# zhm1205/Multimodal_TTA

Measured on AMD Instinct MI355X. Metric: adapted volumes/sec, higher is better.
Workload: dtype bf16

## Files before the change

include/mmtta.h:

```cpp
#ifndef MMTTA_H
#define MMTTA_H

#include <stdint.h>

#ifdef __cplusplus
extern "C" {
#endif

#define MMTTA_ABI_VERSION 2

typedef enum {
  MMTTA_OK = 0,
  MMTTA_ERR_INVALID = -1,
  MMTTA_ERR_UNSUPPORTED = -2,
  MMTTA_ERR_LAUNCH = -3,
  MMTTA_ERR_WORKSPACE = -4
} mmtta_status;

typedef enum { MMTTA_F32 = 0, MMTTA_BF16 = 1 } mmtta_dtype;

typedef struct {
  void* ptr;
  int32_t n, c, d, h, w;
  int64_t sn, sc, sd, sh, sw;
// ... 9 lines not shown
typedef struct {
  const float* mean;
  const float* rstd;
  const float* gamma;
  const float* beta;
  int32_t relu;
  int32_t per_item;
  const float* scale;
  const float* shift;
  float negative_slope;
  int32_t _pad2;
} mmtta_norm_on_load;

const char* mmtta_last_error(void);
int mmtta_abi_version(void);

#define MMTTA_OPT_PROFILE_MAIN_KERNEL_ONLY 1
#define MMTTA_OPT_SPLITK_BELOW 2
#define MMTTA_OPT_SPLITK_TARGET 3
#define MMTTA_OPT_WGRAD_WORKGROUPS 4
#define MMTTA_OPT_WGRAD_THIN_SLABS 5
#define MMTTA_OPT_IGEMM_PIPELINE 6
#define MMTTA_OPT_EPILOGUE_VEC16 9
#define MMTTA_OPT_IGEMM_LEAN 10
#define MMTTA_OPT_WGRAD_VECTOR_STAGING 11
#define MMTTA_OPT_CLASS_FUSED_MIN_WORKGROUPS 12
#define MMTTA_OPT_THIN_MFMA 13
#define MMTTA_OPT_IGEMM_FRAGMENT_REUSE 14
#define MMTTA_OPT_LAME_TILED 15
#define MMTTA_OPT_RAW_STAGING 16
#define MMTTA_OPT_HEAD_LOSS_PAIR 17
#define MMTTA_OPT_THIN_LEAN 18
#define MMTTA_OPT_WGRAD_EPILOGUE_UPDATE 19
int mmtta_set_option(int key, int value);

int mmtta_copy_strided(const mmtta_tensor* src, const mmtta_tensor* dst, void* stream);

typedef enum {
  MMTTA_CONV_FWD = 0,
  MMTTA_CONV_DGRAD = 1,
  MMTTA_CONVT_FWD = 2,
  MMTTA_CONVT_DGRAD = 3
} mmtta_conv_op;

typedef struct {
  int32_t op;
  int32_t ksize;
  int32_t stride;
  int32_t cin;
  int32_t cout;
  int32_t dtype;
} mmtta_conv_desc;

int64_t mmtta_conv_packed_bytes(const mmtta_conv_desc* desc);

int mmtta_conv_pack_weights(const mmtta_conv_desc* desc, const float* w_master, void* packed, void* stream);

typedef struct {
  mmtta_conv_desc desc;
  const float* w_master;
  void* packed;
} mmtta_pack_item;
int64_t mmtta_conv_pack_table_bytes(int count);
int mmtta_conv_pack_table_build(const mmtta_pack_item* items, int count, void* table_host, int64_t* total);
int mmtta_conv_pack_batched(const void* table_dev, int count, int64_t total, void* stream);

typedef struct {
  int32_t tiles;
  int32_t launches;
  int32_t ksplit;
  int32_t stats_rows;
  int32_t config;
  int32_t _pad;
  int64_t workspace_bytes;
} mmtta_conv_plan_t;

int mmtta_conv_plan(const mmtta_conv_desc* desc, const mmtta_tensor* x, const mmtta_tensor* y,
                    mmtta_conv_plan_t* plan);

typedef struct {
  const mmtta_tensor* add;
  mmtta_norm_on_load add_norm;
} mmtta_conv_epilogue;

int mmtta_conv_run(const mmtta_conv_desc* desc, const mmtta_tensor* x, const mmtta_norm_on_load* x_norm,
                   const void* packed, const float* bias, const mmtta_conv_epilogue* epi,
                   const mmtta_tensor* y, int accumulate, float* stats, void* workspace,
                   int64_t workspace_bytes, void* stream);

int mmtta_conv_route(const mmtta_conv_desc* desc, const mmtta_tensor* x, const mmtta_norm_on_load* x_norm,
                     const mmtta_conv_epilogue* epi, const mmtta_tensor* y, int accumulate, const float* stats);

int mmtta_conv_stages_raw(const mmtta_conv_desc* desc, const mmtta_tensor* x, const mmtta_norm_on_load* x_norm,
                          const mmtta_conv_epilogue* epi, const mmtta_tensor* y, int accumulate, const float* stats);

int mmtta_conv_thin_lean(const mmtta_conv_desc* desc, const mmtta_tensor* x, const mmtta_norm_on_load* x_norm,
                         const mmtta_conv_epilogue* epi, const mmtta_tensor* y, int accumulate, const float* stats);

typedef struct {
  int32_t items_per_set;
  int32_t inner;
  int64_t packed_outer, packed_inner;
  int64_t weight_outer, weight_inner;
  int64_t bias_outer, bias_inner;
} mmtta_param_sets;

int mmtta_conv_run_sets(const mmtta_conv_desc* desc, const mmtta_tensor* x, const mmtta_norm_on_load* x_norm,
                        const void* packed, const float* bias, const mmtta_conv_epilogue* epi,
                        const mmtta_tensor* y, int accumulate, float* stats, void* workspace,
                        int64_t workspace_bytes, const mmtta_param_sets* sets, void* stream);

int mmtta_conv_head_loss_eligible(const mmtta_conv_desc* desc, const mmtta_tensor* x, const mmtta_norm_on_load* x_norm,
                                  const mmtta_conv_epilogue* epi, const mmtta_tensor* y, const mmtta_tensor* dlogits,
                                  int softmax, int per_item);
int64_t mmtta_conv_head_loss_partials(const mmtta_conv_desc* desc, const mmtta_tensor* x, const mmtta_tensor* y);
int mmtta_conv_head_loss_run_sets(const mmtta_conv_desc* desc, const mmtta_tensor* x, const mmtta_norm_on_load* x_norm,
                                  const void* packed, const float* bias, const mmtta_conv_epilogue* epi,
                                  const mmtta_tensor* y, const mmtta_tensor* dlogits, int softmax, int per_item,
                                  double* partial, float* loss, const mmtta_param_sets* sets, void* stream);

int64_t mmtta_conv_wgrad_workspace_bytes(const mmtta_conv_desc* desc, const mmtta_tensor* x,
                                         const mmtta_tensor* dy);
int mmtta_conv_wgrad_kernel(const mmtta_conv_desc* desc, const mmtta_tensor* x, const mmtta_tensor* dy);
int mmtta_conv_wgrad_stages_raw(const mmtta_conv_desc* desc, const mmtta_tensor* x, const mmtta_norm_on_load* x_norm,
                                const mmtta_tensor* dy);
int mmtta_conv_wgrad(const mmtta_conv_desc* desc, const mmtta_tensor* x, const mmtta_norm_on_load* x_norm,
                     const mmtta_tensor* dy, float* dw, float* db, int accumulate, void* workspace,
// ... 319 lines not shown
```

multimodal_tta_amd/_lib.py:

```python
from __future__ import annotations

import ctypes as C
import os
from typing import Optional, Sequence

import torch

_HERE = os.path.dirname(os.path.abspath(__file__))
LIB_PATH = os.path.join(_HERE, "csrc", "libmmtta.so")

F32, BF16 = 0, 1
CONV_FWD, CONV_DGRAD, CONVT_FWD, CONVT_DGRAD = 0, 1, 2, 3
NORM_INSTANCE, NORM_BATCH, NORM_GROUP = 0, 1, 2


class MmttaError(RuntimeError):
    pass


class Tensor(C.Structure):
    _fields_ = [
        ("ptr", C.c_void_p),
        ("n", C.c_int32), ("c", C.c_int32), ("d", C.c_int32), ("h", C.c_int32), ("w", C.c_int32),
        ("sn", C.c_int64), ("sc", C.c_int64), ("sd", C.c_int64), ("sh", C.c_int64), ("sw", C.c_int64),
# ... 73 lines not shown


class IntensityRule(C.Structure):
    _fields_ = [("clip", C.c_int32), ("zscore", C.c_int32), ("masked", C.c_int32), ("min_count", C.c_int32),
                ("lo", C.c_float), ("hi", C.c_float), ("mask_gt", C.c_float), ("eps", C.c_float),
                ("mean", C.c_float), ("std", C.c_float), ("legacy", C.c_int32), ("_pad", C.c_int32)]


class InputNormBranch(C.Structure):
    _fields_ = [("dy", C.POINTER(Tensor)), ("weight", C.c_void_p), ("set_stride", C.c_int64), ("ksize", C.c_int32),
                ("stride", C.c_int32)]


_P = C.POINTER
_SIGNATURES = {
    "mmtta_last_error": (C.c_char_p, []),
    "mmtta_abi_version": (C.c_int, []),
    "mmtta_set_option": (C.c_int, [C.c_int, C.c_int]),
    "mmtta_intensity_scratch_bytes": (C.c_int64, [C.c_int]),
    "mmtta_intensity_normalize": (C.c_int, [_P(Tensor), _P(IntensityRule), _P(Tensor), C.c_void_p, C.c_void_p]),
    "mmtta_copy_strided": (C.c_int, [_P(Tensor), _P(Tensor), C.c_void_p]),
    "mmtta_conv_packed_bytes": (C.c_int64, [_P(ConvDesc)]),
    "mmtta_conv_pack_weights": (C.c_int, [_P(ConvDesc), C.c_void_p, C.c_void_p, C.c_void_p]),
    "mmtta_conv_pack_table_bytes": (C.c_int64, [C.c_int]),
    "mmtta_conv_pack_table_build": (C.c_int, [_P(PackItem), C.c_int, C.c_void_p, _P(C.c_int64)]),
    "mmtta_conv_pack_batched": (C.c_int, [C.c_void_p, C.c_int, C.c_int64, C.c_void_p]),
    "mmtta_conv_plan": (C.c_int, [_P(ConvDesc), _P(Tensor), _P(Tensor), _P(ConvPlan)]),
    "mmtta_conv_run": (C.c_int, [_P(ConvDesc), _P(Tensor), _P(NormOnLoad), C.c_void_p, C.c_void_p, _P(ConvEpilogue),
                                 _P(Tensor), C.c_int, C.c_void_p, C.c_void_p, C.c_int64, C.c_void_p]),
    "mmtta_conv_run_sets": (C.c_int, [_P(ConvDesc), _P(Tensor), _P(NormOnLoad), C.c_void_p, C.c_void_p, _P(ConvEpilogue),
                                      _P(Tensor), C.c_int, C.c_void_p, C.c_void_p, C.c_int64, _P(ParamSets), C.c_void_p]),
    "mmtta_conv_route": (C.c_int, [_P(ConvDesc), _P(Tensor), _P(NormOnLoad), _P(ConvEpilogue), _P(Tensor), C.c_int, C.c_void_p]),
    "mmtta_conv_stages_raw": (C.c_int, [_P(ConvDesc), _P(Tensor), _P(NormOnLoad), _P(ConvEpilogue), _P(Tensor), C.c_int, C.c_void_p]),
    "mmtta_conv_thin_lean": (C.c_int, [_P(ConvDesc), _P(Tensor), _P(NormOnLoad), _P(ConvEpilogue), _P(Tensor), C.c_int, C.c_void_p]),
    "mmtta_conv_head_loss_eligible": (C.c_int, [_P(ConvDesc), _P(Tensor), _P(NormOnLoad), _P(ConvEpilogue), _P(Tensor), _P(Tensor),
                                                C.c_int, C.c_int]),
    "mmtta_conv_head_loss_partials": (C.c_int64, [_P(ConvDesc), _P(Tensor), _P(Tensor)]),
    "mmtta_conv_head_loss_run_sets": (C.c_int, [_P(ConvDesc), _P(Tensor), _P(NormOnLoad), C.c_void_p, C.c_void_p, _P(ConvEpilogue),
                                                _P(Tensor), _P(Tensor), C.c_int, C.c_int, C.c_void_p, C.c_void_p, _P(ParamSets),
                                                C.c_void_p]),
    "mmtta_conv_wgrad_workspace_bytes": (C.c_int64, [_P(ConvDesc), _P(Tensor), _P(Tensor)]),
    "mmtta_conv_wgrad_workspace_bytes_sets": (C.c_int64, [_P(ConvDesc), _P(Tensor), _P(Tensor), _P(ParamSets)]),
    "mmtta_conv_wgrad_plan_sets": (C.c_int, [_P(ConvDesc), _P(Tensor), _P(Tensor), _P(ParamSets), _P(C.c_int32)]),
    "mmtta_conv_wgrad_sets": (C.c_int, [_P(ConvDesc), _P(Tensor), _P(NormOnLoad), _P(Tensor), C.c_void_p, C.c_void_p,
                                        C.c_int, C.c_void_p, C.c_int64, _P(ParamSets), C.c_void_p]),
    "mmtta_conv_wgrad_kernel": (C.c_int, [_P(ConvDesc), _P(Tensor), _P(Tensor)]),
    "mmtta_conv_wgrad_stages_raw": (C.c_int, [_P(ConvDesc), _P(Tensor), _P(NormOnLoad), _P(Tensor)]),
    "mmtta_conv_wgrad": (C.c_int, [_P(ConvDesc), _P(Tensor), _P(NormOnLoad), _P(Tensor), C.c_void_p, C.c_void_p,
                                   C.c_int, C.c_void_p, C.c_int64, C.c_void_p]),
    "mmtta_norm_stats_finalize": (C.c_int, [C.c_int, C.c_int, C.c_void_p, C.c_int, C.c_int, C.c_int, C.c_int64,
                                            C.c_float, C.c_int, C.c_void_p, C.c_void_p, C.c_float, C.c_void_p,
                                            C.c_void_p, C.c_void_p, C.c_void_p, C.c_void_p, C.c_void_p, C.c_void_p,
                                            C.c_void_p]),
    "mmtta_norm_stats_finalize_sets": (C.c_int, [C.c_int, C.c_int, C.c_void_p, C.c_int, C.c_int, C.c_int, C.c_int64,
                                                 C.c_float, C.c_int, C.c_void_p, C.c_void_p, C.c_float, C.c_void_p,
                                                 C.c_void_p, C.c_void_p, C.c_void_p, C.c_void_p, C.c_void_p, C.c_void_p,
                                                 C.c_void_p, C.c_void_p, _P(NormSets), C.c_void_p]),
    "mmtta_reduce_rows_per_n": (C.c_int, [_P(Tensor)]),
    "mmtta_channel_stats": (C.c_int, [_P(Tensor), C.c_void_p, C.c_void_p]),
    "mmtta_combine": (C.c_int, [_P(Tensor), _P(NormOnLoad), _P(Tensor), _P(NormOnLoad), _P(Tensor), C.c_void_p]),
    "mmtta_norm_bwd_reduce": (C.c_int, [_P(Tensor), _P(Tensor), _P(NormOnLoad), C.c_void_p, C.c_void_p]),
    "mmtta_norm_bwd_finalize": (C.c_int, [C.c_int, C.c_int, C.c_void_p, C.c_int, C.c_int, C.c_int, C.c_int64,
                                          C.c_void_p, C.c_int, C.c_void_p, C.c_void_p, C.c_void_p, C.c_void_p,
                                          C.c_int, C.c_void_p, C.c_void_p]),
    "mmtta_norm_bwd_finalize_sets": (C.c_int, [C.c_int, C.c_int, C.c_void_p, C.c_int, C.c_int, C.c_int, C.c_int64,
                                               C.c_void_p, C.c_int, C.c_void_p, C.c_void_p, C.c_void_p, C.c_void_p,
# ... 128 lines not shown
        return _lib
    if not os.path.exists(LIB_PATH):
        raise MmttaError(
            f"{LIB_PATH} is missing: build it with `python -m multimodal_tta_amd.build` (hipcc, gfx950). "
            "There is no CPU or PyTorch fallback for the adaptation path."
        )
    lib = C.CDLL(LIB_PATH)
    for name, (res, args) in _SIGNATURES.items():
        fn = getattr(lib, name)
        fn.restype = res
        fn.argtypes = args
    if lib.mmtta_abi_version() != 2:
        raise MmttaError("libmmtta.so ABI version mismatch")
    if os.environ.get("MMTTA_NO_PIPE", "0") == "1":
        lib.mmtta_set_option(6, 0)
    if os.environ.get("MMTTA_NO_EPIVEC", "0") == "1":
        lib.mmtta_set_option(9, 0)
    if "MMTTA_WGVEC" in os.environ:
        lib.mmtta_set_option(11, int(os.environ["MMTTA_WGVEC"]))
    if "MMTTA_THINMFMA" in os.environ:
        lib.mmtta_set_option(13, int(os.environ["MMTTA_THINMFMA"]))
    if "MMTTA_CLSFUSE" in os.environ:
        lib.mmtta_set_option(12, int(os.environ["MMTTA_CLSFUSE"]))
    if "MMTTA_LEAN" in os.environ:
        lib.mmtta_set_option(10, int(os.environ["MMTTA_LEAN"]))
    if "MMTTA_RAWSTAGE" in os.environ:
        lib.mmtta_set_option(16, int(os.environ["MMTTA_RAWSTAGE"]))
    if "MMTTA_HEADLOSS" in os.environ:
        lib.mmtta_set_option(17, int(os.environ["MMTTA_HEADLOSS"]))
    if "MMTTA_THINLEAN" in os.environ:
        lib.mmtta_set_option(18, int(os.environ["MMTTA_THINLEAN"]))
    if "MMTTA_EPIUPDATE" in os.environ:
        lib.mmtta_set_option(19, int(os.environ["MMTTA_EPIUPDATE"]))
    _lib = lib
    return lib


def exported_names() -> Sequence[str]:
    return list(_SIGNATURES)


def check(status: int, what: str = "") -> None:
    if status != 0:
        msg = load().mmtta_last_error().decode("utf-8", "replace")
        raise MmttaError(f"{what or 'libmmtta'} failed with status {status}: {msg}")


def stream_ptr() -> int:
    return int(torch.cuda.current_stream().cuda_stream)


def ptr(t: Optional[torch.Tensor]) -> Optional[int]:
    return None if t is None else int(t.data_ptr())


TENSOR_OWNS_PAD = 1


def desc_cl(t: torch.Tensor) -> Tensor:
    if t.dim() != 5 or t.dtype not in (torch.float32, torch.bfloat16) or not t.is_cuda:
        raise MmttaError(f"expected a CUDA float32 / bfloat16 [N,D,H,W,C] view, got {tuple(t.shape)} {t.dtype} {t.device}")
    n, d, h, w, c = t.shape
    sn, sd, sh, sw, sc = t.stride()
    if sc != 1 and c != 1:
        raise MmttaError("activation views must have unit stride along C")
    flags = TENSOR_OWNS_PAD if getattr(t, "_mmtta_owns_pad", False) else 0
# ... 20 lines not shown
```

multimodal_tta_amd/csrc/api.hip:

```cpp
#include "common.h"
#include <string.h>

namespace mmtta {
static thread_local char g_err[512] = "";
void set_error(const char* fmt, ...) {
  va_list ap;
  va_start(ap, fmt);
  vsnprintf(g_err, sizeof(g_err), fmt, ap);
  va_end(ap);
}
int g_profile_main_only = 0;
int g_igemm_pipeline = 1;
int g_epilogue_vec = 1;
int g_igemm_lean = 1;
int g_igemm_reuse = 1;
int g_cls_fused_min = 128;
int g_thin_mfma = 2;
int g_wgrad_vec = 1;
int g_lame_tiled = 1;
int g_raw_staging = 3;
int g_head_loss_pair = 3;
int g_thin_lean = 3;
int g_wgrad_epilogue_update = 1;
int g_tune[4] = {96, 128, 128, 256};
}

extern "C" int mmtta_set_option(int key, int value) {
  if (key == MMTTA_OPT_PROFILE_MAIN_KERNEL_ONLY) {
    const int prev = mmtta::g_profile_main_only;
    mmtta::g_profile_main_only = value;
    return prev;
  }
  if (key == MMTTA_OPT_WGRAD_VECTOR_STAGING) {
    const int prev = mmtta::g_wgrad_vec;
    mmtta::g_wgrad_vec = value ? 1 : 0;
    return prev;
  }
  if (key == MMTTA_OPT_THIN_MFMA) {
    const int prev = mmtta::g_thin_mfma;
    mmtta::g_thin_mfma = value < 0 ? 0 : (value > 3 ? 3 : value);
    return prev;
  }
  if (key == MMTTA_OPT_CLASS_FUSED_MIN_WORKGROUPS) {
    const int prev = mmtta::g_cls_fused_min;
    mmtta::g_cls_fused_min = value < 0 ? 0 : value;
    return prev;
  }
  if (key == MMTTA_OPT_IGEMM_LEAN) {
    const int prev = mmtta::g_igemm_lean;
    mmtta::g_igemm_lean = value ? 1 : 0;
    return prev;
  }
  if (key == MMTTA_OPT_IGEMM_FRAGMENT_REUSE) {
    const int prev = mmtta::g_igemm_reuse;
    mmtta::g_igemm_reuse = value ? 1 : 0;
    return prev;
  }
  if (key == MMTTA_OPT_EPILOGUE_VEC16) {
    const int prev = mmtta::g_epilogue_vec;
    mmtta::g_epilogue_vec = value ? 1 : 0;
    return prev;
  }
  if (key == MMTTA_OPT_LAME_TILED) {
    const int prev = mmtta::g_lame_tiled;
    mmtta::g_lame_tiled = value ? 1 : 0;
    return prev;
  }
  if (key == MMTTA_OPT_RAW_STAGING) {
    const int prev = mmtta::g_raw_staging;
    mmtta::g_raw_staging = value & 3;
    return prev;
  }
  if (key == MMTTA_OPT_HEAD_LOSS_PAIR) {
    const int prev = mmtta::g_head_loss_pair;
    mmtta::g_head_loss_pair = value & 3;
    return prev;
  }
  if (key == MMTTA_OPT_THIN_LEAN) {
    const int prev = mmtta::g_thin_lean;
    mmtta::g_thin_lean = value & 3;
    return prev;
  }
  if (key == MMTTA_OPT_WGRAD_EPILOGUE_UPDATE) {
    const int prev = mmtta::g_wgrad_epilogue_update;
    mmtta::g_wgrad_epilogue_update = value ? 1 : 0;
    return prev;
  }
  if (key == MMTTA_OPT_IGEMM_PIPELINE) {
    const int prev = mmtta::g_igemm_pipeline;
    mmtta::g_igemm_pipeline = value ? 1 : 0;
    return prev;
  }
  if (key >= MMTTA_OPT_SPLITK_BELOW && key <= MMTTA_OPT_WGRAD_THIN_SLABS) {
    if (value < 1) return MMTTA_ERR_INVALID;
    const int prev = mmtta::g_tune[key - MMTTA_OPT_SPLITK_BELOW];
    mmtta::g_tune[key - MMTTA_OPT_SPLITK_BELOW] = value;
    return prev;
  }
  return MMTTA_ERR_INVALID;
}

extern "C" const char* mmtta_last_error(void) { return mmtta::g_err; }
extern "C" int mmtta_abi_version(void) { return MMTTA_ABI_VERSION; }
```

multimodal_tta_amd/csrc/common.h:

```cpp
#pragma once
#include <hip/hip_runtime.h>
#include <type_traits>
#include <stdint.h>
#include <stdio.h>
#include <stdarg.h>
#include "../../include/mmtta.h"

namespace mmtta {

constexpr int WAVE = 64;

void set_error(const char* fmt, ...);

#define MMTTA_CHECK(cond, code, ...)      \
  do {                                    \
    if (!(cond)) {                        \
      ::mmtta::set_error(__VA_ARGS__);    \
      return (code);                      \
    }                                     \
  } while (0)

inline int launch_status(const char* what) {
  hipError_t e = hipGetLastError();
  if (e != hipSuccess) {
    set_error("%s: %s", what, hipGetErrorString(e));
    return MMTTA_ERR_LAUNCH;
  }
  return MMTTA_OK;
}

extern int g_profile_main_only;
extern int g_igemm_pipeline;
extern int g_wgrad_vec;
extern int g_igemm_lean;
extern int g_igemm_reuse;
extern int g_cls_fused_min;
extern int g_lame_tiled;
extern int g_thin_mfma;
extern int g_epilogue_vec;
extern int g_raw_staging;
extern int g_head_loss_pair;
extern int g_thin_lean;
extern int g_wgrad_epilogue_update;
extern int g_tune[4];

inline bool nl_leaky(const mmtta_norm_on_load* t) { return t != nullptr && t->relu == MMTTA_ACT_LEAKY_RELU; }
inline int nl_act_check(const mmtta_norm_on_load* t, const char* what) {
  MMTTA_CHECK(t == nullptr || (t->relu >= MMTTA_ACT_NONE && t->relu <= MMTTA_ACT_LEAKY_RELU), MMTTA_ERR_INVALID,
              "%s: activation code %d (MMTTA_ACT_NONE, _RELU or _LEAKY_RELU)", what, t ? t->relu : 0);
  MMTTA_CHECK(t == nullptr || t->relu != MMTTA_ACT_LEAKY_RELU || __builtin_isfinite(t->negative_slope), MMTTA_ERR_INVALID,
              "%s: LeakyReLU negative_slope must be finite", what);
  return MMTTA_OK;
}

struct PackImageGeo {
  int A, B, T, Kp, Np, kn_is_ba, plain_bf16;
};
int pack_image_geometry(const mmtta_conv_desc* d, PackImageGeo& g);

#define MMTTA_ACT_BODIES                                                                                                    \
  int conv_run_body(const mmtta_conv_desc* d, const mmtta_tensor* x, const mmtta_norm_on_load* x_norm, const void* packed,  \
                    const float* bias, const mmtta_conv_epilogue* epi, const mmtta_tensor* y, int accumulate, float* stats, \
                    void* workspace, int64_t workspace_bytes, const mmtta_param_sets* sets, void* stream);                \
  int conv_wgrad_body(const mmtta_conv_desc* d, const mmtta_tensor* x, const mmtta_norm_on_load* x_norm,                    \
                      const mmtta_tensor* dy, float* dw, float* db, int accumulate, void* workspace,                        \
                      int64_t workspace_bytes, const mmtta_param_sets* sets, void* stream,                                  \
                      const mmtta_update_target* upd);                                                                      \
  int combine_body(const mmtta_tensor* a, const mmtta_norm_on_load* ta, const mmtta_tensor* b,                              \
                   const mmtta_norm_on_load* tb, const mmtta_tensor* out, void* stream);                                    \
  int norm_bwd_reduce_body(const mmtta_tensor* dout, const mmtta_tensor* y, const mmtta_norm_on_load* t, float* part,      \
                           void* stream);                                                                                   \
  int norm_bwd_apply_body(const mmtta_tensor* dout, const mmtta_tensor* y, const mmtta_norm_on_load* t, const float* m1,   \
                          const float* m2, const mmtta_tensor* dy, void* stream);                                           \
  int norm_bwd_small_body(const mmtta_tensor* dout, const mmtta_tensor* y, const mmtta_norm_on_load* t, int64_t count,     \
                          const mmtta_tensor* dy, void* stream);
namespace leaky { MMTTA_ACT_BODIES }
// ... 460 lines not shown
```

multimodal_tta_amd/csrc/conv_igemm.hip:

```cpp
#include "common.h"

namespace mmtta {
MMTTA_ACT_NS_OPEN

typedef float f32x16 __attribute__((ext_vector_type(16)));
typedef __bf16 bf16x8 __attribute__((ext_vector_type(8)));
typedef __bf16 bf16x2 __attribute__((ext_vector_type(2)));

__device__ __forceinline__ unsigned int pack_bf16x2(float lo, float hi) {
  bf16x2 v;
  v[0] = (__bf16)lo;
  v[1] = (__bf16)hi;
  return __builtin_bit_cast(unsigned int, v);
}

struct Taps {
  int n;
  int slab[27];
  signed char dz[27], dy[27], dx[27];
  int zmin, ymin, xmin;
  int zext, yext, xext;
};

struct ClassInfo {
// ... 217 lines not shown
}

template <int NB, int MB, int TZ, int TY, int TX, int KCI, int OCC>
__global__ __launch_bounds__(256, OCC) void igemm_raw_kernel(GArgs a) {
  constexpr bool BF = true, ABF = true, REUSE = false, RAW = true;
#include "conv_igemm_body.h"
}

template <bool ABF>
__global__ __launch_bounds__(256, 3) void igemm_reuse_raw_kernel(GArgs a) {
  constexpr int NB = 1, MB = 2, TZ = 4, TY = 8, TX = 8, KCI = 16, OCC = 3;
  constexpr bool BF = true, REUSE = true, RAW = true;
#include "conv_igemm_body.h"
}

struct ClsTap { int cls, d, slab; };
__host__ __device__ constexpr ClsTap cls_tap(int f) {
  int idx = 0;
  for (int cls = 0; cls < 8; ++cls) {
    const int pz = (cls >> 2) & 1, py = (cls >> 1) & 1, px = cls & 1;
    for (int a = 0; a <= pz; ++a)
      for (int b = 0; b <= py; ++b)
        for (int c = 0; c <= px; ++c) {
          const int kz = pz ? (a == 0 ? 0 : 2) : 1, dz = pz ? (a == 0 ? 1 : 0) : 0;
          const int ky = py ? (b == 0 ? 0 : 2) : 1, dy = py ? (b == 0 ? 1 : 0) : 0;
          const int kx = px ? (c == 0 ? 0 : 2) : 1, dx = px ? (c == 0 ? 1 : 0) : 0;
          if (idx == f) return ClsTap{cls, (dz * 2 + dy) * 2 + dx, (kz * 3 + ky) * 3 + kx};
          ++idx;
        }
  }
  return ClsTap{0, 0, 0};
}

template <int KCI, bool ABF>
__global__ __launch_bounds__(256, 2) void igemm_cls8_kernel(GArgs a) {
  constexpr bool RAW = false;
#include "conv_igemm_cls8_body.h"
}

template <int KCI, bool ABF>
__global__ __launch_bounds__(256, 2) void igemm_cls8_raw_kernel(GArgs a) {
  constexpr bool RAW = true;
#include "conv_igemm_cls8_body.h"
}

template <int KCI, bool ABF, bool RAW = false>
static int launch_cls8_t(const GArgs& a, int tiles, hipStream_t s) {
  constexpr int VS = KCI + 8;
  size_t lds = ((size_t)(5 * 5 * LDS_PITCH_BF16 * VS + 7) / 8 * 8) * 2 + (size_t)27 * (KCI / 8) * 32 * 16;
  const size_t epi = (4 * EPI_TILE_FLOATS + 4 * 2 * 32) * sizeof(float);
  if (lds < epi) lds = epi;
  void (*kern)(GArgs) = igemm_cls8_kernel<KCI, ABF>;
  if constexpr (RAW) kern = igemm_cls8_raw_kernel<KCI, ABF>;
  static bool attr_set = false;
  if (!attr_set) {
    (void)hipFuncSetAttribute((const void*)kern, hipFuncAttributeMaxDynamicSharedMemorySize, 160 * 1024);
    attr_set = true;
  }
  hipLaunchKernelGGL(kern, dim3(tiles, a.Np / 32), dim3(256), lds, s, a);
  return launch_status("conv igemm (class-fused stride-2 form)");
}

template <int TZ, int TY, int TX, bool PERM, bool ABF = false>
__global__ __launch_bounds__(256) void splitk_finalize_kernel(GArgs a, int tiles) {
  __shared__ float red[2][8][32];
  constexpr int MT = TZ * TY * TX;
  constexpr int RB = MT / 32;
  const int tid = threadIdx.x, r = tid & 31, rg = tid >> 5;
  const int tile = blockIdx.x / RB, rb = blockIdx.x % RB;
  int cidx, t;
  class_of_tile(a, tile, cidx, t);
  const ClassInfo ci = a.cls[cidx];
  const int tile_in_n = t % (a.tz * a.ty * a.tx);
  const int txi = t % a.tx; t /= a.tx;
  const int tyi = t % a.ty; t /= a.ty;
  const int tzi = t % a.tz;
  const int n = t / a.tz;
  const int col = blockIdx.y * 32 + r;
  const bool colok = col < a.Co;
  float bias = 0.f, asc = 1.f, ash = 0.f;
  if (colok) {
    const float* biasn = pset_bias(a.ps, a.bias, n);
    if (biasn) bias = biasn[col];
    if (a.add) nl_coeff(a.tadd, n, a.Co, col, asc, ash);
  }
  float s_sum = 0.f, s_sq = 0.f;
// ... 473 lines not shown
  else if (c.NB == 2) id = c.MB == 4 ? 1 : 4;
  else id = c.KCI == 32 ? 2 : 5;
  return c.bf ? id + 7 : id;
}

enum CRoute : int {
  C_DIRECT = 6,
  C_THIN = 13,
  C_CLS_FUSED = 15,
  C_PW_SMALL = 16,
  C_PW_MFMA = 17,
  C_IGEMM_REUSE = 18,
};

struct RunFacts {
  const float* stats; const mmtta_tensor* add; const mmtta_norm_on_load* x_norm;
  int accumulate;
  const float* bias;
};

#ifdef MMTTA_ACT_LEAKY_TU
constexpr bool RAW_KERNELS = false;
#else
constexpr bool RAW_KERNELS = true;
#endif
static bool raw_operand(const mmtta_tensor* x, const mmtta_norm_on_load* x_norm) {
  return is_bf16(x) && x->c % 8 == 0 && quad_aligned(x, 16, 8) &&
         (x_norm == nullptr || (x_norm->mean == nullptr && x_norm->scale == nullptr && x_norm->relu == MMTTA_ACT_NONE));
}
static bool raw_staging(int route, bool bf_tile, const mmtta_tensor* x, const mmtta_norm_on_load* x_norm, const mmtta_tensor* y,
                        const mmtta_tensor* add) {
  const bool igemm = route != 6 && route != 13 && route != 16 && route != 17;
  return RAW_KERNELS && (g_raw_staging & 1) && igemm && bf_tile && raw_operand(x, x_norm) && is_bf16(y) && (add == nullptr || is_bf16(add));
}

struct Geometry {
  int route;
  int K, N, Kp, Np, si;
  bool classes;
  Config cfg;
  int tz, ty, tx, tiles_per_n, tiles, ncls;
  int nstages, ksplit, sps;
  int stats_rows;
  int64_t workspace_bytes;
};

static int expected_out_dim(const mmtta_conv_desc* d, int in) {
  switch (d->op) {
    case MMTTA_CONV_FWD: return d->stride == 1 ? in : (in + 1) / 2;
    case MMTTA_CONVT_FWD: return in * 2;
    case MMTTA_CONVT_DGRAD: return in / 2;
    default: return -1;
  }
}

static bool pointwise_mfma_applicable(const mmtta_conv_desc* d, const mmtta_tensor* x, const mmtta_tensor* y, const Geometry& g,
                                      const RunFacts& rt) {
  static const bool pw_on = !(getenv("MMTTA_POINTWISE_MFMA") && atoi(getenv("MMTTA_POINTWISE_MFMA")) == 0);
  const int kb = (g.K + 15) / 16;
  auto rows_ok = [&](const mmtta_tensor* t) { return dense_rows16(t) && is_bf16(t) == is_bf16(x); };
  return pw_on && d->ksize == 1 && (d->op == MMTTA_CONV_FWD || d->op == MMTTA_CONV_DGRAD) && use_bf16(d, g.K) &&
         (kb <= 4 || kb == 6 || kb == 8) && g.Np <= 64 && rt.stats == nullptr && !(rt.x_norm && (rt.x_norm->mean || rt.x_norm->scale)) &&
         (long long)y->d * y->h * y->w >= 4096 && rows_ok(x) && rows_ok(y) && (rt.add == nullptr || (rows_ok(rt.add) && same_shape(rt.add, y)));
}

static bool rowload_operand(const mmtta_tensor* x) {
// ... 263 lines not shown
    ci.tap0 = tap0; ci.ntaps = ht[cls].n; tap0 += ht[cls].n;
    ci.zmin = ht[cls].zmin; ci.ymin = ht[cls].ymin; ci.xmin = ht[cls].xmin;
    ci.zext = ht[cls].zext; ci.yext = ht[cls].yext; ci.xext = ht[cls].xext;
    if (g.classes) {
      ci.oz = pz; ci.oy = py; ci.ox = px;
      ci.Dg = (y->d - pz + 1) / 2; ci.Hg = (y->h - py + 1) / 2; ci.Wg = (y->w - px + 1) / 2;
    } else {
      ci.oz = ci.oy = ci.ox = 0;
      ci.Dg = y->d; ci.Hg = y->h; ci.Wg = y->w;
    }
  }
  return MMTTA_OK;
}

static int igemm_run(const ConvCall& c, const Geometry& g) {
  MMTTA_CHECK(g.workspace_bytes == 0 || (c.workspace != nullptr && c.workspace_bytes >= g.workspace_bytes), MMTTA_ERR_WORKSPACE,
              "conv: workspace %lld bytes, need %lld", (long long)c.workspace_bytes, (long long)g.workspace_bytes);
  GArgs a; Taps ht[8];
  const int st = fill_gargs(c, g, a, ht);
  if (st) return st;
  const bool raw = raw_staging(g.route, g.cfg.bf, c.x, c.x_norm, c.y, (c.epi && c.epi->add) ? c.epi->add : nullptr);
  return launch_any(g.route, a, ht, g.tiles, raw, c.stream);
}

static int cls_fused_run(const ConvCall& c, const Geometry& g) {
  GArgs a; Taps ht[8];
  const int st = fill_gargs(c, g, a, ht);
  if (st) return st;
  MMTTA_CHECK(a.ovec && a.vec4, MMTTA_ERR_UNSUPPORTED,
              "conv (class-fused stride-2 form): the epilogue operands must admit 16-byte accesses");
  MMTTA_CHECK(a.in_bf == a.out_bf && (a.add == nullptr || a.add_bf == a.out_bf), MMTTA_ERR_UNSUPPORTED,
              "conv: input, output and fused add must share one storage type (in %d out %d add %d)", a.in_bf, a.out_bf, a.add_bf);
  if constexpr (RAW_KERNELS) {
    if (raw_staging(g.route, g.cfg.bf, c.x, c.x_norm, c.y, (c.epi && c.epi->add) ? c.epi->add : nullptr))
      return launch_cls8_t<16, true, true>(a, g.tiles, c.stream);
  }
  return a.in_bf ? launch_cls8_t<16, true>(a, g.tiles, c.stream) : launch_cls8_t<16, false>(a, g.tiles, c.stream);
}

static int pointwise_mfma_run(const ConvCall& c, const Geometry& g) {
  const mmtta_tensor *x = c.x, *y = c.y, *ad = (c.epi && c.epi->add) ? c.epi->add : nullptr;
  PWArgs q;
  q.in = (const float*)x->ptr; q.isn = x->sn; q.isw = (unsigned)x->sw; q.Ci = x->c;
  q.out = (float*)y->ptr; q.osn = y->sn; q.osw = (unsigned)y->sw; q.Co = y->c;
  q.add = ad ? (const float*)ad->ptr : nullptr; q.asn = ad ? ad->sn : 0; q.asw = ad ? (unsigned)ad->sw : 0u;
  q.tadd = ad ? nl(&c.epi->add_norm) : nl(nullptr);
  q.wp = (const float*)c.packed; q.bias = c.bias; q.Np = g.Np; q.ps = c.ps; q.accumulate = c.accumulate;
  q.dhw = (long long)y->d * y->h * y->w;
  long long blocks = (q.dhw + 127) / 128;
  if (blocks > 2048) blocks = 2048;
  const dim3 grid((unsigned)blocks, y->n);
  if (is_bf16(x)) launch_pointwise_mfma<true>(q, (g.K + 15) / 16, g.Np / 32, grid, c.stream);
  else launch_pointwise_mfma<false>(q, (g.K + 15) / 16, g.Np / 32, grid, c.stream);
  return launch_status("1x1 conv (streaming MFMA)");
}

static int plan_run(const mmtta_conv_desc* d, const mmtta_tensor* x, const mmtta_norm_on_load* x_norm, const mmtta_conv_epilogue* epi,
                    const mmtta_tensor* y, int accumulate, const float* stats, const float* bias, Geometry& g) {
  const RunFacts rt{stats, epi ? epi->add : nullptr, x_norm, accumulate, bias};
  return geometry(d, x, y, &rt, g);
}

int conv_run_body(const mmtta_conv_desc* d, const mmtta_tensor* x, const mmtta_norm_on_load* x_norm, const void* packed,
                  const float* bias, const mmtta_conv_epilogue* epi, const mmtta_tensor* y, int accumulate, float* stats,
                  void* workspace, int64_t workspace_bytes, const mmtta_param_sets* sets, void* stream) {
  Geometry g;
  int st = plan_run(d, x, x_norm, epi, y, accumulate, stats, bias, g);
  if (st) return st;
// ... 114 lines not shown
  int st = launch_status("pack batched");
  if (st) return st;
  hipLaunchKernelGGL(pack_chan_frags_batched_kernel, dim3((unsigned)count), dim3(256), 0, (hipStream_t)stream, (const PackEntry*)table_dev);
  return launch_status("pack batched (thin-K fragments)");
}

extern "C" int mmtta_conv_plan(const mmtta_conv_desc* d, const mmtta_tensor* x, const mmtta_tensor* y,
                               mmtta_conv_plan_t* plan) {
  MMTTA_CHECK(plan != nullptr, MMTTA_ERR_INVALID, "conv plan: null plan");
  Geometry g;
  int st = geometry(d, x, y, nullptr, g);
  if (st) return st;
  *plan = mmtta_conv_plan_t{g.tiles,  1, g.ksplit, g.stats_rows, g.route, 0, g.workspace_bytes};
  return MMTTA_OK;
}

extern "C" int mmtta_conv_route(const mmtta_conv_desc* d, const mmtta_tensor* x, const mmtta_norm_on_load* x_norm,
                                const mmtta_conv_epilogue* epi, const mmtta_tensor* y, int accumulate, const float* stats) {
  Geometry g;
  const int st = plan_run(d, x, x_norm, epi, y, accumulate, stats, nullptr, g);
  if (st) return st < 0 ? st : -st;
  return g.route;
}

extern "C" int mmtta_conv_stages_raw(const mmtta_conv_desc* d, const mmtta_tensor* x, const mmtta_norm_on_load* x_norm,
                                     const mmtta_conv_epilogue* epi, const mmtta_tensor* y, int accumulate, const float* stats) {
  Geometry g;
  const int st = plan_run(d, x, x_norm, epi, y, accumulate, stats, nullptr, g);
  if (st) return st < 0 ? st : -st;
  const mmtta_tensor* add = (epi && epi->add) ? epi->add : nullptr;
  return (raw_staging(g.route, g.cfg.bf, x, x_norm, y, add) && !(add && nl_leaky(&epi->add_norm))) ? 1 : 0;
}

extern "C" int mmtta_conv_thin_lean(const mmtta_conv_desc* d, const mmtta_tensor* x, const mmtta_norm_on_load* x_norm,
                                    const mmtta_conv_epilogue* epi, const mmtta_tensor* y, int accumulate, const float* stats) {
  Geometry g;
  const int st = plan_run(d, x, x_norm, epi, y, accumulate, stats, nullptr, g);
  if (st) return st < 0 ? st : -st;
  if (g.route == C_THIN) return chan_lean_applicable(d, x, x_norm, epi, y, accumulate) ? 1 : 0;
  if (g.route == C_DIRECT) return direct_upconv8_lean(d, x, x_norm, epi, y) ? 2 : 0;
  return 0;
}

static int head_loss_plan(const mmtta_conv_desc* d, const mmtta_tensor* x, const mmtta_norm_on_load* x_norm,
                          const mmtta_conv_epilogue* epi, const mmtta_tensor* y, const mmtta_tensor* dz, int softmax, int per_item,
                          bool& eligible) {
  Geometry g;
  const int st = plan_run(d, x, x_norm, epi, y, 0, nullptr, nullptr, g);
  if (st) return st;
  eligible = g.route == C_DIRECT && direct_head_loss_eligible(d, x, x_norm, epi, y, dz, softmax, per_item);
  return MMTTA_OK;
}

extern "C" int mmtta_conv_head_loss_eligible(const mmtta_conv_desc* d, const mmtta_tensor* x, const mmtta_norm_on_load* x_norm,
                                             const mmtta_conv_epilogue* epi, const mmtta_tensor* y, const mmtta_tensor* dlogits,
                                             int softmax, int per_item) {
  bool ok = false;
  const int st = head_loss_plan(d, x, x_norm, epi, y, dlogits, softmax, per_item, ok);
  if (st) return st < 0 ? st : -st;
  return ok ? 1 : 0;
}

extern "C" int64_t mmtta_conv_head_loss_partials(const mmtta_conv_desc* d, const mmtta_tensor* x, const mmtta_tensor* y) {
  Geometry g;
  if (geometry(d, x, y, nullptr, g) || g.route != C_DIRECT) return -1;
  return (int64_t)direct_blocks_per_n(d, x, y) * y->n;
// ... 54 lines not shown
```

multimodal_tta_amd/csrc/conv_igemm_cls8_body.h:

```cpp
  constexpr int TZ = 4, TY = 4, TX = 8, VS = KCI + 8, LP = LDS_PITCH_BF16, KS = KCI / 16, KC8 = KCI / 8;
  constexpr int BZ = TZ + 1, BY = TY + 1, BX = TX + 1;
  constexpr int BOX_HW = BZ * BY * LP * VS;
  constexpr int WIMG = 27 * KC8 * 32;
  extern __shared__ float lds[];
  unsigned short* lh = reinterpret_cast<unsigned short*>(lds);
  uint4* wimg = reinterpret_cast<uint4*>(lh + (BOX_HW + 7) / 8 * 8);
  const int tid = threadIdx.x, lane = tid & 63;
  const int wave = __builtin_amdgcn_readfirstlane(tid >> 6);
  const int h = lane >> 5, r = lane & 31;
  int t = blockIdx.x;
  const int tile_in_n = t % (a.tz * a.ty * a.tx);
  const int txi = t % a.tx; t /= a.tx;
  const int tyi = t % a.ty; t /= a.ty;
  const int tzi = t % a.tz;
  const int n = t / a.tz;
  const float* biasn = pset_bias(a.ps, a.bias, n);
  const int gz0 = tzi * TZ, gy0 = tyi * TY, gx0 = txi * TX;
  const int colbase = blockIdx.y * 32;
  const bool colact = colbase < a.Np;

  int zl, yl, xl;
  row_to_local<TZ, TY, TX, true>(wave * 32 + r, zl, yl, xl);
  const unsigned short* arow = lh + ((zl * BY + yl) * LP + xl) * VS + 8 * h;
  const uint4* brow = wimg + h * 32 + r;

  f32x16 acc[8];
#pragma unroll
  for (int c = 0; c < 8; ++c)
#pragma unroll
    for (int i = 0; i < 16; ++i) acc[c][i] = 0.f;

  const uint4* wq = reinterpret_cast<const uint4*>(pset_packed(a.ps, a.wp, n));
  const long long slabsz8 = (long long)(a.Kp / 8) * a.Np;
  const unsigned isd = (unsigned)a.isd, ish = (unsigned)a.ish, isw = (unsigned)a.isw;
  const int cmax = ABF ? ((a.Ci - 1) & ~7) : ((a.Ci - 1) & ~3);
  constexpr int AIT = (BZ * BY * BX * KC8 + 255) / 256;
  constexpr int BIT = (WIMG + 255) / 256;
  const float relu_lo = act_lo(a.tin.relu);

  for (int ks = 0; ks < a.nstages; ++ks) {
    const int c0 = ks * KCI;
    const float* sb = reinterpret_cast<const float*>(reinterpret_cast<const char*>(a.in) + ((long long)n * a.isn + c0) * (ABF ? 2 : 4));
    uint4 wv[BIT];
#pragma unroll
    for (int j = 0; j < BIT; ++j) {
      const int i = min(tid + 256 * j, WIMG - 1);
      const int tap = i / (KC8 * 32), rem = i - tap * (KC8 * 32), k8l = rem >> 5, col = rem & 31;
      wv[j] = wq[tap * slabsz8 + (long long)(c0 / 8 + k8l) * a.Np + colbase + col];
    }
    Oct8<ABF> av[AIT];
    unsigned aok = 0u;
    int alds[AIT];
#pragma unroll
    for (int j = 0; j < AIT; ++j) {
      const int i = min(tid + 256 * j, BZ * BY * BX * KC8 - 1);
      const int cv = i % KC8, bv = i / KC8;
      const int bz = bv / (BY * BX), brem = bv - bz * (BY * BX), by = brem / BX, bx = brem - by * BX;
      const int iz = gz0 + bz, iy = gy0 + by, ix = gx0 + bx;
      bool ok = iz < a.Di && iy < a.Hi && ix < a.Wi;
      if constexpr (RAW) ok = ok && c0 + cv * 8 < a.Ci;
      aok |= (ok ? 1u : 0u) << j;
      const unsigned off = __umul24((unsigned)min(iz, a.Di - 1), isd) + __umul24((unsigned)min(iy, a.Hi - 1), ish) +
                           __umul24((unsigned)min(ix, a.Wi - 1), isw) + cv * 8;
      const int over = max(c0 + cv * 8 - cmax, 0), over_hi = max(c0 + cv * 8 + 4 - cmax, 0);
      av[j] = oct8_ld<ABF>(sb, off - over, off + 4 - over_hi);
      alds[j] = ((bz * BY + by) * LP + bx) * VS + cv * 8;
    }
    float sc[AIT][8], sh[AIT][8];
    if constexpr (!RAW) {
#pragma unroll
    for (int j = 0; j < AIT; ++j) {
      const int i = min(tid + 256 * j, BZ * BY * BX * KC8 - 1);
      nl_coeff_vec<8>(a.tin, n, a.Ci, c0 + (i % KC8) * 8, sc[j], sh[j]);
    }
    }
#pragma unroll
    for (int j = 0; j < BIT; ++j)
      if (tid + 256 * j < WIMG) wimg[tid + 256 * j] = wv[j];
#pragma unroll
    for (int j = 0; j < AIT; ++j) {
      const unsigned okm = ((aok >> j) & 1u) ? 0xffffffffu : 0u;
      uint4 pk;
      if constexpr (RAW) {
        pk = av[j].q;
        pk.x &= okm; pk.y &= okm; pk.z &= okm; pk.w &= okm;
      } else {
      float v[8];
      oct8_f8(av[j], v);
#pragma unroll
      for (int q = 0; q < 8; ++q) v[q] = act_max(fmaf(v[q], sc[j][q], sh[j][q]), relu_lo);
      pk.x = pack_bf16x2(v[0], v[1]) & okm; pk.y = pack_bf16x2(v[2], v[3]) & okm;
      pk.z = pack_bf16x2(v[4], v[5]) & okm; pk.w = pack_bf16x2(v[6], v[7]) & okm;
      }
      if (tid + 256 * j < BZ * BY * BX * KC8) *reinterpret_cast<uint4*>(lh + alds[j]) = pk;
    }
    __syncthreads();
    if (colact) {
#pragma unroll
      for (int k16 = 0; k16 < KS; ++k16) {
        uint4 af[8];
#pragma unroll
        for (int d = 0; d < 8; ++d)
          af[d] = *reinterpret_cast<const uint4*>(arow + ((((d >> 2) & 1) * BY + ((d >> 1) & 1)) * LP + (d & 1)) * VS + k16 * 16);
        constexpr int LA = 3;
        uint4 bring[LA + 1];
        static_for<0, LA>([&](auto fc) {
          constexpr int f = decltype(fc)::value;
          bring[f] = brow[(cls_tap(f).slab * KC8 + k16 * 2) * 32];
        });
        __builtin_amdgcn_sched_barrier(0);
        static_for<0, 27>([&](auto fc) {
          constexpr int f = decltype(fc)::value;
          constexpr ClsTap ct = cls_tap(f);
          if constexpr (f + LA < 27) bring[(f + LA) % (LA + 1)] = brow[(cls_tap(f + LA).slab * KC8 + k16 * 2) * 32];
          acc[ct.cls] = __builtin_amdgcn_mfma_f32_32x32x16_bf16(__builtin_bit_cast(bf16x8, af[ct.d]),
                                                                __builtin_bit_cast(bf16x8, bring[f % (LA + 1)]), acc[ct.cls], 0, 0, 0);
          __builtin_amdgcn_sched_barrier(0);
        });
      }
    }
    __syncthreads();
  }
  float tsum[4] = {0.f, 0.f, 0.f, 0.f}, tsq[4] = {0.f, 0.f, 0.f, 0.f};
#pragma unroll
  for (int c = 0; c < 8; ++c) {
    float v_sum[4], v_sq[4];
    epilogue_vec16<TZ, TY, TX, 1, true, ABF>(a, biasn, a.cls[c], *reinterpret_cast<f32x16(*)[1]>(&acc[c]), lds + wave * EPI_TILE_FLOATS,
                                             lane, wave, colbase, colact, n, gz0, gy0, gx0, v_sum, v_sq);
#pragma unroll
    for (int j = 0; j < 4; ++j) { tsum[j] += v_sum[j]; tsq[j] += v_sq[j]; }
  }
  if (a.stats != nullptr) {
    float* red = lds + 4 * EPI_TILE_FLOATS;
    if (lane < 8) {
#pragma unroll
      for (int j = 0; j < 4; ++j) {
        red[(wave * 2 + 0) * 32 + lane * 4 + j] = tsum[j];
        red[(wave * 2 + 1) * 32 + lane * 4 + j] = tsq[j];
      }
    }
    __syncthreads();
    const int col = colbase + tid;
    if (tid < 32 && col < a.Co) {
      float ts = 0.f, tq = 0.f;
#pragma unroll
      for (int g = 0; g < 4; ++g) { ts += red[(g * 2 + 0) * 32 + tid]; tq += red[(g * 2 + 1) * 32 + tid]; }
      const long long row = (long long)n * a.stats_rows_per_n + tile_in_n;
// ... 5 lines not shown
```

Measured before the change: 120.3.

## Add double-buffered pipelined cls8 igemm kernel with async weight loads to LDS

```diff
diff --git a/include/mmtta.h b/include/mmtta.h
--- a/include/mmtta.h
+++ b/include/mmtta.h
@@ -65,6 +65,7 @@
 #define MMTTA_OPT_HEAD_LOSS_PAIR 17
 #define MMTTA_OPT_THIN_LEAN 18
 #define MMTTA_OPT_WGRAD_EPILOGUE_UPDATE 19
+#define MMTTA_OPT_CLS8_PIPELINE 20
 int mmtta_set_option(int key, int value);
 
 int mmtta_copy_strided(const mmtta_tensor* src, const mmtta_tensor* dst, void* stream);
@@ -126,6 +127,9 @@
 
 int mmtta_conv_stages_raw(const mmtta_conv_desc* desc, const mmtta_tensor* x, const mmtta_norm_on_load* x_norm,
                           const mmtta_conv_epilogue* epi, const mmtta_tensor* y, int accumulate, const float* stats);
+
+int mmtta_conv_cls8_pipelined(const mmtta_conv_desc* desc, const mmtta_tensor* x, const mmtta_norm_on_load* x_norm,
+                              const mmtta_conv_epilogue* epi, const mmtta_tensor* y, int accumulate, const float* stats);
 
 int mmtta_conv_thin_lean(const mmtta_conv_desc* desc, const mmtta_tensor* x, const mmtta_norm_on_load* x_norm,
                          const mmtta_conv_epilogue* epi, const mmtta_tensor* y, int accumulate, const float* stats);
diff --git a/multimodal_tta_amd/_lib.py b/multimodal_tta_amd/_lib.py
--- a/multimodal_tta_amd/_lib.py
+++ b/multimodal_tta_amd/_lib.py
@@ -129,6 +129,7 @@
                                       _P(Tensor), C.c_int, C.c_void_p, C.c_void_p, C.c_int64, _P(ParamSets), C.c_void_p]),
     "mmtta_conv_route": (C.c_int, [_P(ConvDesc), _P(Tensor), _P(NormOnLoad), _P(ConvEpilogue), _P(Tensor), C.c_int, C.c_void_p]),
     "mmtta_conv_stages_raw": (C.c_int, [_P(ConvDesc), _P(Tensor), _P(NormOnLoad), _P(ConvEpilogue), _P(Tensor), C.c_int, C.c_void_p]),
+    "mmtta_conv_cls8_pipelined": (C.c_int, [_P(ConvDesc), _P(Tensor), _P(NormOnLoad), _P(ConvEpilogue), _P(Tensor), C.c_int, C.c_void_p]),
     "mmtta_conv_thin_lean": (C.c_int, [_P(ConvDesc), _P(Tensor), _P(NormOnLoad), _P(ConvEpilogue), _P(Tensor), C.c_int, C.c_void_p]),
     "mmtta_conv_head_loss_eligible": (C.c_int, [_P(ConvDesc), _P(Tensor), _P(NormOnLoad), _P(ConvEpilogue), _P(Tensor), _P(Tensor),
                                                 C.c_int, C.c_int]),
@@ -323,6 +324,8 @@
         lib.mmtta_set_option(18, int(os.environ["MMTTA_THINLEAN"]))
     if "MMTTA_EPIUPDATE" in os.environ:
         lib.mmtta_set_option(19, int(os.environ["MMTTA_EPIUPDATE"]))
+    if "MMTTA_CLS8PIPE" in os.environ:
+        lib.mmtta_set_option(20, int(os.environ["MMTTA_CLS8PIPE"]))
     _lib = lib
     return lib
 
diff --git a/multimodal_tta_amd/csrc/api.hip b/multimodal_tta_amd/csrc/api.hip
--- a/multimodal_tta_amd/csrc/api.hip
+++ b/multimodal_tta_amd/csrc/api.hip
@@ -22,6 +22,7 @@
 int g_head_loss_pair = 3;
 int g_thin_lean = 3;
 int g_wgrad_epilogue_update = 1;
+int g_cls8_pipeline = 1;
 int g_tune[4] = {96, 128, 128, 256};
 }
 
@@ -86,6 +87,11 @@
     mmtta::g_wgrad_epilogue_update = value ? 1 : 0;
     return prev;
   }
+  if (key == MMTTA_OPT_CLS8_PIPELINE) {
+    const int prev = mmtta::g_cls8_pipeline;
+    mmtta::g_cls8_pipeline = value ? 1 : 0;
+    return prev;
+  }
   if (key == MMTTA_OPT_IGEMM_PIPELINE) {
     const int prev = mmtta::g_igemm_pipeline;
     mmtta::g_igemm_pipeline = value ? 1 : 0;
diff --git a/multimodal_tta_amd/csrc/common.h b/multimodal_tta_amd/csrc/common.h
--- a/multimodal_tta_amd/csrc/common.h
+++ b/multimodal_tta_amd/csrc/common.h
@@ -42,6 +42,7 @@
 extern int g_head_loss_pair;
 extern int g_thin_lean;
 extern int g_wgrad_epilogue_update;
+extern int g_cls8_pipeline;
 extern int g_tune[4];
 
 inline bool nl_leaky(const mmtta_norm_on_load* t) { return t != nullptr && t->relu == MMTTA_ACT_LEAKY_RELU; }
diff --git a/multimodal_tta_amd/csrc/conv_igemm.hip b/multimodal_tta_amd/csrc/conv_igemm.hip
--- a/multimodal_tta_amd/csrc/conv_igemm.hip
+++ b/multimodal_tta_amd/csrc/conv_igemm.hip
@@ -273,26 +273,44 @@
   return ClsTap{0, 0, 0};
 }
 
+typedef unsigned cls8_u32x4 __attribute__((ext_vector_type(4)));
+template <bool TYPED>
+__device__ __forceinline__ uint4 cls8_lds_q(const void* p) {
+  if constexpr (TYPED) {
+    const cls8_u32x4 v = *reinterpret_cast<const cls8_u32x4*>(p);
+    return make_uint4(v.x, v.y, v.z, v.w);
+  } else {
+    return *reinterpret_cast<const uint4*>(p);
+  }
+}
+
 template <int KCI, bool ABF>
 __global__ __launch_bounds__(256, 2) void igemm_cls8_kernel(GArgs a) {
-  constexpr bool RAW = false;
+  constexpr bool RAW = false, PIPE = false;
 #include "conv_igemm_cls8_body.h"
 }
 
 template <int KCI, bool ABF>
 __global__ __launch_bounds__(256, 2) void igemm_cls8_raw_kernel(GArgs a) {
-  constexpr bool RAW = true;
+  constexpr bool RAW = true, PIPE = false;
 #include "conv_igemm_cls8_body.h"
 }
 
-template <int KCI, bool ABF, bool RAW = false>
+template <int KCI, bool ABF>
+__global__ __launch_bounds__(256, 2) void igemm_cls8_pipe_kernel(GArgs a) {
+  constexpr bool RAW = true, PIPE = true;
+#include "conv_igemm_cls8_body.h"
+}
+
+template <int KCI, bool ABF, bool RAW = false, bool PIPE = false>
 static int launch_cls8_t(const GArgs& a, int tiles, hipStream_t s) {
   constexpr int VS = KCI + 8;
-  size_t lds = ((size_t)(5 * 5 * LDS_PITCH_BF16 * VS + 7) / 8 * 8) * 2 + (size_t)27 * (KCI / 8) * 32 * 16;
+  size_t lds = ((size_t)(5 * 5 * LDS_PITCH_BF16 * VS + 7) / 8 * 8) * 2 + (size_t)(PIPE ? 2 : 1) * 27 * (KCI / 8) * 32 * 16;
   const size_t epi = (4 * EPI_TILE_FLOATS + 4 * 2 * 32) * sizeof(float);
   if (lds < epi) lds = epi;
   void (*kern)(GArgs) = igemm_cls8_kernel<KCI, ABF>;
-  if constexpr (RAW) kern = igemm_cls8_raw_kernel<KCI, ABF>;
+  if constexpr (RAW && !PIPE) kern = igemm_cls8_raw_kernel<KCI, ABF>;
+  if constexpr (PIPE) kern = igemm_cls8_pipe_kernel<KCI, ABF>;
   static bool attr_set = false;
   if (!attr_set) {
     (void)hipFuncSetAttribute((const void*)kern, hipFuncAttributeMaxDynamicSharedMemorySize, 160 * 1024);
@@ -832,6 +850,11 @@
                         const mmtta_tensor* add) {
   const bool igemm = route != 6 && route != 13 && route != 16 && route != 17;
   return RAW_KERNELS && (g_raw_staging & 1) && igemm && bf_tile && raw_operand(x, x_norm) && is_bf16(y) && (add == nullptr || is_bf16(add));
+}
+
+static bool cls8_pipelined(int route, bool bf_tile, const mmtta_tensor* x, const mmtta_norm_on_load* x_norm, const mmtta_tensor* y,
+                           const mmtta_tensor* add) {
+  return g_cls8_pipeline && route == 15  && raw_staging(route, bf_tile, x, x_norm, y, add);
 }
 
 struct Geometry {
@@ -1161,8 +1184,9 @@
   MMTTA_CHECK(a.in_bf == a.out_bf && (a.add == nullptr || a.add_bf == a.out_bf), MMTTA_ERR_UNSUPPORTED,
               "conv: input, output and fused add must share one storage type (in %d out %d add %d)", a.in_bf, a.out_bf, a.add_bf);
   if constexpr (RAW_KERNELS) {
-    if (raw_staging(g.route, g.cfg.bf, c.x, c.x_norm, c.y, (c.epi && c.epi->add) ? c.epi->add : nullptr))
-      return launch_cls8_t<16, true, true>(a, g.tiles, c.stream);
+    const mmtta_tensor* ad = (c.epi && c.epi->add) ? c.epi->add : nullptr;
+    if (cls8_pipelined(g.route, g.cfg.bf, c.x, c.x_norm, c.y, ad)) return launch_cls8_t<16, true, true, true>(a, g.tiles, c.stream);
+    if (raw_staging(g.route, g.cfg.bf, c.x, c.x_norm, c.y, ad)) return launch_cls8_t<16, true, true>(a, g.tiles, c.stream);
   }
   return a.in_bf ? launch_cls8_t<16, true>(a, g.tiles, c.stream) : launch_cls8_t<16, false>(a, g.tiles, c.stream);
 }
@@ -1343,6 +1367,15 @@
   return (raw_staging(g.route, g.cfg.bf, x, x_norm, y, add) && !(add && nl_leaky(&epi->add_norm))) ? 1 : 0;
 }
 
+extern "C" int mmtta_conv_cls8_pipelined(const mmtta_conv_desc* d, const mmtta_tensor* x, const mmtta_norm_on_load* x_norm,
+                                         const mmtta_conv_epilogue* epi, const mmtta_tensor* y, int accumulate, const float* stats) {
+  Geometry g;
+  const int st = plan_run(d, x, x_norm, epi, y, accumulate, stats, nullptr, g);
+  if (st) return st < 0 ? st : -st;
+  const mmtta_tensor* add = (epi && epi->add) ? epi->add : nullptr;
+  return (cls8_pipelined(g.route, g.cfg.bf, x, x_norm, y, add) && !(add && nl_leaky(&epi->add_norm))) ? 1 : 0;
+}
+
 extern "C" int mmtta_conv_thin_lean(const mmtta_conv_desc* d, const mmtta_tensor* x, const mmtta_norm_on_load* x_norm,
                                     const mmtta_conv_epilogue* epi, const mmtta_tensor* y, int accumulate, const float* stats) {
   Geometry g;
diff --git a/multimodal_tta_amd/csrc/conv_igemm_cls8_body.h b/multimodal_tta_amd/csrc/conv_igemm_cls8_body.h
--- a/multimodal_tta_amd/csrc/conv_igemm_cls8_body.h
+++ b/multimodal_tta_amd/csrc/conv_igemm_cls8_body.h
@@ -38,7 +38,65 @@
   constexpr int BIT = (WIMG + 255) / 256;
   const float relu_lo = act_lo(a.tin.relu);
 
+  static_assert(!PIPE || (RAW && ABF && KC8 * 32 == 64 && WIMG % 64 == 0), "the pipelined form: raw staging of 16-channel stages");
+  unsigned wlane = 0u;
+  unsigned poff[AIT], phalo = 0u;
+  auto pipe_cv8 = [&](int j) { return (min(tid + 256 * j, BZ * BY * BX * KC8 - 1) % KC8) * 8; };
+  int plds[AIT];
+  Oct8<ABF> pav[AIT];
+  if constexpr (PIPE) {
+    wlane = (unsigned)((lane >> 5) * a.Np + colbase + (lane & 31)) * 16u;
+#pragma unroll
+    for (int j = 0; j < AIT; ++j) {
+      const int i = min(tid + 256 * j, BZ * BY * BX * KC8 - 1);
+      const int cv = i % KC8, bv = i / KC8;
+      const int bz = bv / (BY * BX), brem = bv - bz * (BY * BX), by = brem / BX, bx = brem - by * BX;
+      const int iz = gz0 + bz, iy = gy0 + by, ix = gx0 + bx;
+      phalo |= ((iz < a.Di && iy < a.Hi && ix < a.Wi) ? 1u : 0u) << j;
+      poff[j] = __umul24((unsigned)min(iz, a.Di - 1), isd) + __umul24((unsigned)min(iy, a.Hi - 1), ish) +
+                __umul24((unsigned)min(ix, a.Wi - 1), isw) + cv * 8;
+      plds[j] = ((bz * BY + by) * LP + bx) * VS + cv * 8;
+    }
+  }
+  auto pipe_issue = [&](int ks) {
+    if constexpr (PIPE) {
+    const char* src = reinterpret_cast<const char*>(wq + (long long)ks * KC8 * a.Np);
+    uint4* dst = wimg + (ks & 1) * WIMG + 64 * wave;
+#pragma unroll
+    for (int j = 0; j < BIT; ++j)
+      if (j < BIT - 1 || 256 * j + 64 * wave < WIMG)
+        __builtin_amdgcn_global_load_lds((const __attribute__((address_space(1))) void*)(src + (long long)(4 * j + wave) * slabsz8 * 16 + wlane),
+                                         (__attribute__((address_space(3))) void*)(dst + 256 * j), 16, 0, 0);
+    const int c0 = ks * KCI;
+    const float* sb = reinterpret_cast<const float*>(reinterpret_cast<const char*>(a.in) + ((long long)n * a.isn + c0) * 2);
+#pragma unroll
+    for (int j = 0; j < AIT; ++j) {
+      const int over = max(c0 + pipe_cv8(j) - cmax, 0);
+      pav[j] = oct8_ld<ABF>(sb, poff[j] - over, 0u);
+    }
+    }
+  };
+  auto pipe_commit = [&](int ks) {
+    if constexpr (PIPE) {
+#pragma unroll
+    for (int j = 0; j < AIT; ++j) {
+      const unsigned okm = (((phalo >> j) & 1u) && ks * KCI + pipe_cv8(j) < a.Ci) ? 0xffffffffu : 0u;
+      uint4 pk = pav[j].q;
+      pk.x &= okm; pk.y &= okm; pk.z &= okm; pk.w &= okm;
+      if (tid + 256 * j < BZ * BY * BX * KC8) *reinterpret_cast<uint4*>(lh + plds[j]) = pk;
+    }
+    }
+  };
+  if constexpr (PIPE) {
+    __builtin_assume(a.nstages > 0);
+    pipe_issue(0);
+  }
+
   for (int ks = 0; ks < a.nstages; ++ks) {
+    const uint4* const bst = PIPE ? brow + (ks & 1) * WIMG : brow;
+    if constexpr (PIPE) {
+      pipe_commit(ks);
+    } else {
     const int c0 = ks * KCI;
     const float* sb = reinterpret_cast<const float*>(reinterpret_cast<const char*>(a.in) + ((long long)n * a.isn + c0) * (ABF ? 2 : 4));
     uint4 wv[BIT];
@@ -94,25 +152,29 @@
       }
       if (tid + 256 * j < BZ * BY * BX * KC8) *reinterpret_cast<uint4*>(lh + alds[j]) = pk;
     }
+    }
     __syncthreads();
+    if constexpr (PIPE) {
+      if (ks + 1 < a.nstages) pipe_issue(ks + 1);
+    }
     if (colact) {
 #pragma unroll
       for (int k16 = 0; k16 < KS; ++k16) {
         uint4 af[8];
 #pragma unroll
         for (int d = 0; d < 8; ++d)
-          af[d] = *reinterpret_cast<const uint4*>(arow + ((((d >> 2) & 1) * BY + ((d >> 1) & 1)) * LP + (d & 1)) * VS + k16 * 16);
+          af[d] = cls8_lds_q<PIPE>(arow + ((((d >> 2) & 1) * BY + ((d >> 1) & 1)) * LP + (d & 1)) * VS + k16 * 16);
         constexpr int LA = 3;
         uint4 bring[LA + 1];
         static_for<0, LA>([&](auto fc) {
           constexpr int f = decltype(fc)::value;
-          bring[f] = brow[(cls_tap(f).slab * KC8 + k16 * 2) * 32];
+          bring[f] = cls8_lds_q<PIPE>(bst + (cls_tap(f).slab * KC8 + k16 * 2) * 32);
         });
         __builtin_amdgcn_sched_barrier(0);
         static_for<0, 27>([&](auto fc) {
           constexpr int f = decltype(fc)::value;
           constexpr ClsTap ct = cls_tap(f);
-          if constexpr (f + LA < 27) bring[(f + LA) % (LA + 1)] = brow[(cls_tap(f + LA).slab * KC8 + k16 * 2) * 32];
+          if constexpr (f + LA < 27) bring[(f + LA) % (LA + 1)] = cls8_lds_q<PIPE>(bst + (cls_tap(f + LA).slab * KC8 + k16 * 2) * 32);
           acc[ct.cls] = __builtin_amdgcn_mfma_f32_32x32x16_bf16(__builtin_bit_cast(bf16x8, af[ct.d]),
                                                                 __builtin_bit_cast(bf16x8, bring[f % (LA + 1)]), acc[ct.cls], 0, 0, 0);
           __builtin_amdgcn_sched_barrier(0);
```

Measured after the change: 121.8 (median of 6 runs). 1.01x the previous value.
